# Nuralamsiddik16/Ultrafnd_git

Measured on AMD Instinct MI355X. Metric: train-step samples/sec (FakeSV batch, seq128+224^2), higher is better.
Workload: dtype bf16

## Files before the change

include/ultrafnd_hip.h:

```cpp
#ifndef ULTRAFND_HIP_H
#define ULTRAFND_HIP_H

#include <stddef.h>
#include <stdint.h>

#ifdef __cplusplus
extern "C" {
#endif

#define UFND_OK 0
#define UFND_ERR_INVALID 1
#define UFND_ERR_LAUNCH 2

#define UFND_ABI_VERSION 6

const char* ufnd_last_error(void);
int ufnd_abi_version(void);

typedef struct ufnd_step_state {
  uint64_t step;
  uint64_t seed;
  float lr;
  float weight_decay;
  float beta1, beta2, eps;
// ... 165 lines not shown
int ufnd_attention_bf16(const void* qkv, const int32_t* key_mask, void* ctx, int B, int L, int heads,
                        void* stream);

int ufnd_qkv_attention_bf16(const void* X, const void* Wqkv, const float* bqkv, const int32_t* key_mask, void* ctx, int B, int L,
                            int heads, int ldx, int ldw, const ufnd_gemm_ln* ln, void* stream);

int ufnd_text_pack(const int32_t* mask, int B, int L, int32_t* cu_seqlens, int32_t* row_src, void* stream);
int ufnd_text_pack_bins(const int32_t* mask, int B, int L, int32_t* cu_seqlens, int32_t* row_src, int32_t* bins, int32_t* nbins,
                        void* stream);
int ufnd_bert_embed_live(const int64_t* ids, const int32_t* row_src, const int* m_live, const float* word, const float* pos,
                         const float* type0, const float* gamma, const float* beta, void* x_bf16, float* x_f32, int capacity, int L,
                         int H, int vocab, float eps, void* stream);
int ufnd_gemm_bf16_live(const void* A, const void* W, const float* bias, const float* residual, void* out_bf16, float* out_f32,
                        int M, int N, int K, int lda, int ldw, int ldr, int ldo, int ldf, int act, int tile_cfg, const int* m_live,
                        void* stream);
int ufnd_gemm_bf16_ln_live(const void* A, const void* W, const float* bias, const float* residual, void* out_bf16, float* out_f32,
                           int M, int N, int K, int lda, int ldw, int ldr, int ldo, int ldf, int act, const ufnd_gemm_ln* ln,
                           const int* m_live, void* stream);
int ufnd_qkv_attention_bf16_packed(const void* X, const void* Wqkv, const float* bqkv, const int32_t* key_mask, const int32_t* cu_seqlens,
                                   void* ctx, int B, int L, int heads, int ldx, int ldw, const ufnd_gemm_ln* ln, void* stream);
int ufnd_qkv_attention_bf16_bins(const void* X, const void* Wqkv, const float* bqkv, const int32_t* key_mask, const int32_t* cu_seqlens,
                                 const int32_t* bins, const int32_t* nbins, void* ctx, int B, int L, int heads, int ldx, int ldw,
                                 const ufnd_gemm_ln* ln, void* stream);
int ufnd_attention_bf16_varlen_masked(const void* qkv, const int32_t* cu_seqlens, const int32_t* key_mask, void* ctx, int B, int max_len,
                                      int heads, void* stream);

int ufnd_qkv_attention_bf16_vit(const void* X, const void* Wqkv, const float* bqkv, void* ctx, int N, int T, int heads, int ldx, int ldw,
                                const ufnd_gemm_ln* ln, void* stream);
int ufnd_layernorm_live(const float* x, int ldx, const float* gamma, const float* beta, void* out_bf16, float* out_f32, int capacity,
                        int H, float eps, const int* m_live, void* stream);
int ufnd_masked_meanpool_l2_live(const float* hidden, const int32_t* mask, const int32_t* cu_seqlens, float* out, int B, int L, int H,
                                 void* stream);

int ufnd_bert_embed(const int64_t* ids, const float* word, const float* pos, const float* type0, const float* gamma,
                    const float* beta, void* x_bf16, float* x_f32, int B, int L, int H, int vocab, float eps,
                    void* stream);

int ufnd_masked_meanpool_l2(const float* hidden, const int32_t* mask, float* out, int B, int L, int H,
                            void* stream);

int ufnd_field_mean_l2(const float* parts, const int32_t* valid, float* out, int N, int M, int D, void* stream);

int ufnd_vit_patchify(const float* frames, void* patches_bf16, int N, int image, int patch, void* stream);

int ufnd_vit_assemble(const float* patch_emb, const float* cls, const float* pos, const float* gamma,
                      const float* beta, float* x_f32, void* x_bf16, float* stats, int N, int P, int H, float eps,
// ... 214 lines not shown
```

ultrafnd_git_amd/_lib.py:

```python
from __future__ import annotations

import ctypes as C
from pathlib import Path
from typing import Optional

import torch

_PKG = Path(__file__).resolve().parent
LIB_PATH = _PKG / "libultrafnd_hip.so"


class UltrafndHipError(RuntimeError):
    pass


class StepState(C.Structure):
    _fields_ = [("step", C.c_uint64), ("seed", C.c_uint64), ("lr", C.c_float), ("weight_decay", C.c_float),
                ("beta1", C.c_float), ("beta2", C.c_float), ("eps", C.c_float), ("max_norm", C.c_float),
                ("grad_scale", C.c_float), ("loss", C.c_float), ("grad_norm", C.c_float), ("clip_coef", C.c_float),
                ("bc1", C.c_float), ("bc2_sqrt", C.c_float), ("micro", C.c_uint32), ("reserved", C.c_float * 2)]


class Dims(C.Structure):
    _fields_ = [("hidden", C.c_int), ("text_dim", C.c_int), ("audio_dim", C.c_int), ("visual_dim", C.c_int),
# ... 127 lines not shown
                 "ufnd_softmax_ce", "ufnd_grad_norm", "ufnd_adamw_step", "ufnd_step_advance"):
        getattr(lib, name).restype = I
    _declare_encoders(lib)


def _declare_encoders(lib: C.CDLL) -> None:
    P, I, S, F = C.c_void_p, C.c_int, C.c_size_t, C.c_float
    sigs = {
        "ufnd_cast_bf16": [P, P, S, P],
        "ufnd_gemm_bf16": [P] * 6 + [I] * 9 + [P],
        "ufnd_gemm_bf16_ex": [P] * 6 + [I] * 10 + [P],
        "ufnd_layernorm": [P, I, P, P, P, P, I, I, F, P],
        "ufnd_attention_bf16": [P, P, P, I, I, I, P],
        "ufnd_qkv_attention_bf16": [P, P, P, P, P, I, I, I, I, I, C.POINTER(GemmLn), P],
        "ufnd_bert_embed": [P] * 8 + [I, I, I, I, F, P],
        "ufnd_masked_meanpool_l2": [P, P, P, I, I, I, P],
        "ufnd_text_pack": [P, I, I, P, P, P],
        "ufnd_text_pack_bins": [P, I, I, P, P, P, P, P],
        "ufnd_bert_embed_live": [P] * 10 + [I, I, I, I, F, P],
        "ufnd_gemm_bf16_live": [P] * 6 + [I] * 10 + [P, P],
        "ufnd_gemm_bf16_ln_live": [P] * 6 + [I] * 9 + [C.POINTER(GemmLn), P, P],
        "ufnd_qkv_attention_bf16_packed": [P, P, P, P, P, P, I, I, I, I, I, C.POINTER(GemmLn), P],
        "ufnd_qkv_attention_bf16_bins": [P] * 8 + [I, I, I, I, I, C.POINTER(GemmLn), P],
        "ufnd_qkv_attention_bf16_vit": [P, P, P, P, I, I, I, I, I, C.POINTER(GemmLn), P],
        "ufnd_attention_bf16_varlen_masked": [P, P, P, P, I, I, I, P],
        "ufnd_layernorm_live": [P, I, P, P, P, P, I, I, F, P, P],
        "ufnd_masked_meanpool_l2_live": [P, P, P, P, I, I, I, P],
        "ufnd_vit_patchify": [P, P, I, I, I, P],
        "ufnd_vit_assemble": [P] * 8 + [I, I, I, F, P],
        "ufnd_gemm_bf16_ln": [P] * 6 + [I] * 9 + [C.POINTER(GemmLn), P],
        "ufnd_gemm_bf16_stat_parts": [I, I, I],
        "ufnd_ln_fold_guard": [P, I, I, I, F, P, P],
        "ufnd_gemm_bf16_tile_count": [],
        "ufnd_gemm_bf16_tile_info": [I, C.POINTER(I), C.POINTER(I), C.POINTER(I)],
        "ufnd_stream_create_cu_mask": [C.POINTER(C.c_uint32), I, C.POINTER(P)],
        "ufnd_stream_destroy": [P],
        "ufnd_device_cu_count": [],
        "ufnd_l2norm_frames": [P, P, I, I, I, P],
        "ufnd_field_mean_l2": [P, P, P, I, I, I, P],
        "ufnd_temporal_align": [P] * 8 + [I] * 5 + [F, P, P],
    }
    sigs.update({
        "ufnd_gemm_bf16_dgrad": [P] * 6 + [I] * 10 + [P],
        "ufnd_gemm_bf16_wgrad": [P, P, P, I, I, I, I, I, I, P, I, P],
        "ufnd_transpose_bf16": [P, I, I, I, I, P, I, I, P, P, I, P],
        "ufnd_linear_wgrad": [P, I, P, I, I, I, I, P, P, P, P, I, P, P, C.POINTER(PartialsJob), I, P],
# ... 141 lines not shown
```

ultrafnd_git_amd/csrc/gemm_bf16.hip:

```cpp
#include "gemm_bf16_kernel.hpp"
#include "gemm_bf16_checks.hpp"

#define UFND_GEMM_TILE_PP UFND_GEMM_TILE_PERSISTENT
int ufnd_pp_pick(const void* gemm_args);
int ufnd_pp_launch(void* gemm_args, void* stream);
int ufnd_pp_stat_parts(int N);

namespace {
__global__ __launch_bounds__(256) void cast_bf16_kernel(const float* src, __bf16* dst, size_t n) {
  for (size_t i = (blockIdx.x * (size_t)256 + threadIdx.x) * 4; i < n; i += (size_t)gridDim.x * 256 * 4) {
    if (i + 4 <= n) {
      const f32x4 v = *reinterpret_cast<const f32x4*>(src + i);
      bf16x4 o = {(__bf16)v[0], (__bf16)v[1], (__bf16)v[2], (__bf16)v[3]};
      *reinterpret_cast<bf16x4*>(dst + i) = o;
    } else {
      for (size_t j = i; j < n; ++j) dst[j] = (__bf16)src[j];
    }
  }
}

}

extern "C" int ufnd_gemm_bf16_live(const void* A, const void* W, const float* bias, const float* residual, void* out_bf16,
                                   float* out_f32, int M, int N, int K, int lda, int ldw, int ldr, int ldo, int ldf, int act,
// ... 125 lines not shown
  if (ln && ln->a_stats) {
    UFND_REQUIRE(ln->colsum && ufnd_aligned(ln->colsum, 16) && ufnd_aligned(ln->a_stats, 16), "qkv_attention: colsum / a_stats alignment");
    UFND_REQUIRE(ln->a_parts >= 2 && ln->a_parts <= 24 && ln->a_parts % 2 == 0 && ln->width > 0, "qkv_attention: a_parts=%d width=%d", ln->a_parts, ln->width);
    a.a_stats = ln->a_stats; a.colsum = ln->colsum; a.a_parts = ln->a_parts; a.a_eps = ln->a_eps;
    a.inv_h = 1.0f / (float)ln->width;
    a.guard = ln->guard;
  }
  a.att_mask = key_mask;
  a.att_cu = cu_seqlens;
  a.att_bins = bins;
  a.att_nbins = nbins;
  a.m_live = cu_seqlens ? cu_seqlens + B : nullptr;
  a.att_ctx = (__bf16*)ctx;
  a.att_h = H;
  a.att_scale_log2e = 0.125f * 1.44269504088896340736f;
  a.m_tiles = B;
  a.n_tiles = heads / 2;
  a.xcd_cols = (a.n_tiles % 2 == 0 && a.m_tiles >= 4) ? 2 : 1;
  hipLaunchKernelGGL((gemm_bf16_kernel<128, 384, 2, 4, 3, 2, 16, 0, 0, 1, 1>), dim3(a.m_tiles * a.n_tiles), dim3(512), 0, (hipStream_t)stream_, a);
  UFND_CHECK_LAUNCH();
  return UFND_OK;
}

extern "C" int ufnd_qkv_attention_bf16_vit(const void* X, const void* Wqkv, const float* bqkv, void* ctx, int N, int T, int heads, int ldx,
                                           int ldw, const ufnd_gemm_ln* ln, void* stream_) {
  UFND_REQUIRE(X && Wqkv && ctx, "qkv_attention_vit: null operand");
  UFND_REQUIRE(T >= 1 && T <= 64, "qkv_attention_vit: T=%d (this kernel is built for samples of 1 to 64 rows; use ufnd_gemm_bf16[_ln] + "
               "ufnd_attention_bf16 otherwise)", T);
  UFND_REQUIRE(heads >= 1 && heads <= 64 && N >= 1 && (long long)N * T <= (1 << 24), "qkv_attention_vit: N=%d T=%d heads=%d", N, T, heads);
  const int H = heads * 64;
  UFND_REQUIRE(ldx % 8 == 0 && ldw % 8 == 0 && ldx >= H && ldw >= H && ufnd_aligned(X, 16) && ufnd_aligned(Wqkv, 16) && ufnd_aligned(ctx, 16),
               "qkv_attention_vit: strides must be multiples of 8 and pointers 16-B aligned");
  UFND_REQUIRE(!bqkv || ufnd_aligned(bqkv, 16), "qkv_attention_vit: bias alignment");
  GemmArgs a{(const __bf16*)X, (const __bf16*)Wqkv, bqkv, nullptr, nullptr, nullptr, N * T, 3 * H, H, ldx, ldw, 0, 0, 0, UFND_ACT_NONE, 0, 0, nullptr};
  if (ln && ln->a_stats) {
    UFND_REQUIRE(ln->colsum && ufnd_aligned(ln->colsum, 16) && ufnd_aligned(ln->a_stats, 16), "qkv_attention_vit: colsum / a_stats alignment");
    UFND_REQUIRE(ln->a_parts >= 2 && ln->a_parts <= 24 && ln->a_parts % 2 == 0 && ln->width > 0, "qkv_attention_vit: a_parts=%d width=%d", ln->a_parts, ln->width);
    a.a_stats = ln->a_stats; a.colsum = ln->colsum; a.a_parts = ln->a_parts; a.a_eps = ln->a_eps;
    a.inv_h = 1.0f / (float)ln->width;
    a.guard = ln->guard;
  }
  a.att_ctx = (__bf16*)ctx;
  a.att_h = H;
  a.att_t = T;
  a.att_scale_log2e = 0.125f * 1.44269504088896340736f;
  a.m_tiles = ufnd_cdiv(N, 256 / T);
// ... 23 lines not shown
```

ultrafnd_git_amd/csrc/gemm_bf16_kernel.hpp:

```cpp
#pragma once
#ifndef UFND_GEMM_OUT_NT
#define UFND_GEMM_OUT_NT 0
#endif

#include <type_traits>

#include "common.hpp"
#include "attn_softmax.hpp"

#pragma clang fp contract(off)

#ifndef UFND_GEMM_ILV
#define UFND_GEMM_ILV 1
#endif

namespace {

constexpr int BK = 64;

struct GemmArgs {
  const __bf16* A;
  const __bf16* W;
  const float* bias;
  const float* residual;
// ... 46 lines not shown

__device__ __forceinline__ bf16x8 lds_frag(const char* tile, int row, int chunk) {
  return *reinterpret_cast<const bf16x8*>(tile + row * 128 + ((chunk ^ ((row >> 1) & 7)) << 4));
}

template <int N>
__device__ __forceinline__ void wait_vmcnt() {
  static_assert(N >= 0 && N <= 63, "vmcnt range");
  asm volatile("s_waitcnt vmcnt(%0)" ::"n"(N) : "memory");
}

template <int V> struct IntC { static constexpr int value = V; };

constexpr int gemm_waves_per_simd(int BM, int BN, int WM, int WN, int STA, int STB, int MI, int LNX, int ATT) {
  const int ring = (STA * BM + STB * BN) * 128, cbytes = WM * WN * MI * (BN / WN + 4) * 4;
  const int smem = (ring > cbytes ? ring : cbytes) + (LNX ? BM * 8 + 64 : 0);
  return (!ATT && smem <= 80 * 1024 ? 2 : 1) * WM * WN / 4;
}
template <int BM, int BN, int WM, int WN, int STA, int STB, int MI, int ABL = 0, int DBG = 0, int LNX = 0, int ATT = 0, int BWD = 0>
__global__ __launch_bounds__(WM * WN * 64) __attribute__((amdgpu_waves_per_eu(gemm_waves_per_simd(BM, BN, WM, WN, STA, STB, MI, LNX, ATT))))
void gemm_bf16_kernel(const GemmArgs a) {
  static_assert(!BWD || (!LNX && !ATT && !ABL && !DBG), "backward forms are plain kernels");
  static_assert(MI == 16 || MI == 32, "MFMA shape");
  static_assert(!ATT || (((BM == 128 && BN == 384) || (BM == 256 && BN == 192)) && MI == 16 && WM * WN == 8 && LNX == 1), "fused attention tile");
  constexpr bool VIT = ATT && BM == 256;
  using acc_t = typename std::conditional<MI == 16, f32x4, f32x16>::type;
  constexpr int AR = MI * MI / 64;
  constexpr int KQ = MI == 16 ? 1 : 2;
  constexpr int NW = WM * WN;
  constexpr int TM = BM / WM, TN = BN / WN;
  constexpr int MT = TM / MI, NT = TN / MI;
  constexpr int ASLOT = BM * 128, BSLOT = BN * 128;
  constexpr int DA = STA - 1, DB = STB - 1;
  constexpr int APIECES = BM / 8, BPIECES = BN / 8;
  constexpr int PWA = APIECES / NW, PWB = (BPIECES + NW - 1) / NW;
  constexpr int WAITN = PWA * (DA - 1 > 0 ? DA - 1 : 0) + PWB * (DB - 1 > 0 ? DB - 1 : 0);
  constexpr int CP = TN + 4;
  constexpr int CBYTES = NW * MI * CP * 4;
  constexpr int RING = STA * ASLOT + STB * BSLOT;
  constexpr int ATT_OFF = (CBYTES + 1023) & ~1023;
  constexpr int ATT_IMG = BM * 128;
  constexpr int ATT_END = ATT ? ATT_OFF + (VIT ? 3 * ATT_IMG + 256 : 6 * ATT_IMG + 2048) : 0;
  constexpr int STAT_OFF0 = (RING > CBYTES) ? RING : CBYTES;
  constexpr int STAT_OFF = STAT_OFF0 > ATT_END ? STAT_OFF0 : ATT_END;
  constexpr int SMEM = STAT_OFF + (LNX ? BM * 8 + 64 : 0);
  static_assert(SMEM <= 160 * 1024, "LDS budget");
  static_assert(APIECES % NW == 0 && TM % MI == 0 && TN % MI == 0, "tile split");
  static_assert(STB >= 2 && (STA == STB || STA == STB + 1), "ring depths");
  static_assert(WAITN <= 63, "vmcnt range");
  __shared__ __attribute__((aligned(16))) char smem[SMEM];

  unsigned long long stamp[10];
  if constexpr (DBG) {
    stamp[0] = __builtin_amdgcn_s_memtime();
    stamp[1] = __builtin_amdgcn_s_memrealtime();
  }

  int mlive = a.M, m_tiles = a.m_tiles;
  if constexpr (!BWD && !ATT) {
    if (a.m_live) {
      const int v = __builtin_amdgcn_readfirstlane(*a.m_live);
      mlive = v < a.M ? (v > 0 ? v : 0) : a.M;
      m_tiles = (mlive + BM - 1) / BM;
      if ((int)blockIdx.x >= m_tiles * a.n_tiles) return;
    }
  }
  if constexpr (ATT) {
    if (a.att_bins) {
      const int v = __builtin_amdgcn_readfirstlane(*a.att_nbins);
      m_tiles = v < a.m_tiles ? (v > 0 ? v : 0) : a.m_tiles;
      if ((int)blockIdx.x >= m_tiles * a.n_tiles) return;
    }
  }
  const int nblk = m_tiles * a.n_tiles;
  int bid, kslice = 0;
  {
    const int ngrid = BWD ? nblk * (a.ksplit > 1 ? a.ksplit : 1) : nblk;
    const int q = ngrid >> 3, r = ngrid & 7, xcd = blockIdx.x & 7, idx = blockIdx.x >> 3;
    bid = (xcd < r ? xcd * (q + 1) : r * (q + 1) + (xcd - r) * q) + idx;
    if constexpr (BWD) {
      kslice = bid / nblk;
      bid -= kslice * nblk;
    }
  }
  int tm = bid / a.n_tiles, tn = bid % a.n_tiles;
  if (a.xcd_cols == 2) {
    const int nh = a.n_tiles >> 1, per_half = m_tiles * nh;
    const int half = bid / per_half, rem = bid - half * per_half;
    tm = rem / nh;
    tn = half * nh + (rem - tm * nh);
  }
  const int m0 = tm * BM, n0 = tn * BN;
  int arow0 = m0, alen = BM;
  int srow[4] = {0, 0, 0, 0}, scnt[4] = {0, 0, 0, 0}, smeta[4] = {-1, -1, -1, -1};
  const bool slots = ATT && !VIT && a.att_bins != nullptr;
  const int vit_s = VIT ? BM / a.att_t : 0, vit_st = vit_s * a.att_t;
  if constexpr (VIT) {
    arow0 = tm * vit_st;
    alen = mlive - arow0 < vit_st ? mlive - arow0 : vit_st;
  } else if constexpr (ATT) {
    if (slots) {
      const int32_t* bd = a.att_bins + (size_t)tm * 8;
#pragma unroll
      for (int j = 0; j < 4; ++j) {
        srow[j] = __builtin_amdgcn_readfirstlane(bd[2 * j]);
        smeta[j] = __builtin_amdgcn_readfirstlane(bd[2 * j + 1]);
        const int n = smeta[j] & 255, rest = n - 32 * ((smeta[j] >> 8) & 3);
        scnt[j] = smeta[j] < 0 ? 0 : (rest < 32 ? rest : 32);
      }
#pragma unroll
      for (int j = 1; j < 4; ++j) srow[j] = scnt[j] > 0 ? srow[j] : srow[0];
    } else if (a.att_cu) {
      mlive = __builtin_amdgcn_readfirstlane(*a.m_live);
      arow0 = __builtin_amdgcn_readfirstlane(a.att_cu[tm]);
      alen = __builtin_amdgcn_readfirstlane(a.att_cu[tm + 1]) - arow0;
      if (alen <= 0) return;
    }
  } else {
    alen = mlive - m0;
  }
  auto tile_row = [&](int tr) {
    if (slots) {
      const int j = tr >> 5, q = tr & 31;
      const int r0 = j == 0 ? srow[0] : j == 1 ? srow[1] : j == 2 ? srow[2] : srow[3];
      const int c = j == 0 ? scnt[0] : j == 1 ? scnt[1] : j == 2 ? scnt[2] : scnt[3];
      return r0 + (q < c ? q : (c > 0 ? c - 1 : 0));
    }
    const int gr = arow0 + tr;
    return gr < mlive ? gr : mlive - 1;
  };
  auto tile_row_live = [&](int tr) {
    if (slots) {
      const int j = tr >> 5;
      return (tr & 31) < (j == 0 ? scnt[0] : j == 1 ? scnt[1] : j == 2 ? scnt[2] : scnt[3]);
    }
    return tr < alen;
  };
  const int wave = __builtin_amdgcn_readfirstlane(threadIdx.x >> 6), lane = threadIdx.x & 63;
  const int wm = wave / WN, wn = wave % WN, fr = lane & (MI - 1), g = lane / MI;

  acc_t acc[MT][NT];
#pragma unroll
  for (int i = 0; i < MT; ++i)
#pragma unroll
    for (int j = 0; j < NT; ++j)
#pragma unroll
      for (int r = 0; r < AR; ++r) acc[i][j][r] = 0.f;

  int nk = a.K / BK, kbase = 0;
  if constexpr (BWD) {
    if (a.ksplit > 1) {
      const int per = (nk + a.ksplit - 1) / a.ksplit;
      kbase = kslice * per * BK;
      nk = nk - kslice * per < per ? nk - kslice * per : per;
    }
  }
  const int prow = lane >> 3, ppos = lane & 7;
// ... 7 lines not shown
    const int k0 = kbase + kt * BK;
#pragma unroll
    for (int ii = 0; ii < PWA; ++ii) {
      const int p = wave + NW * ii;
      const int r = 8 * p + prow;
      const int c = ppos ^ ((r >> 1) & 7);
      int gr = arow0 + r;
      gr = gr < mlive ? gr : mlive - 1;
      if constexpr (ATT) gr = arow_att[ii];
      dma16(a.A + (size_t)gr * a.lda + k0 + c * 8, buf + p * 1024);
    }
  };
  auto issueB = [&](int t, int kt) {
    char* buf = smem + STA * ASLOT + (t % STB) * BSLOT;
    const int k0 = kbase + kt * BK;
#pragma unroll
    for (int ii = 0; ii < PWB; ++ii) {
      int p = wave + NW * ii;
      if constexpr (BPIECES % NW != 0) p = p < BPIECES ? p : p - BPIECES;
      const int r = 8 * p + prow;
      const int c = ppos ^ ((r >> 1) & 7);
      int gr = n0 + r;
      gr = gr < a.N ? gr : a.N - 1;
      if constexpr (VIT) gr = (r >> 6) * a.att_h + tn * 64 + (r & 63);
      else if constexpr (ATT) gr = (r >> 7) * a.att_h + tn * 128 + (r & 127);
      dma16(a.W + (size_t)gr * a.ldw + k0 + c * 8, buf + p * 1024);
    }
  };
  constexpr int TPR = NW * 64 / BM;
  static_assert(!LNX || TPR == 2 || TPR == 4, "threads per tile row");
  constexpr int GPT = 4 / (TPR < 4 ? TPR : 4);
  f32x4 sv[GPT][3];
  f32x2* st_lds = reinterpret_cast<f32x2*>(smem + STAT_OFF);
  const float* sp = nullptr;
  if constexpr (LNX) {
    sp = a.a_stats ? a.a_stats : a.r_stats;
    if (sp) {
      const int parts = a.a_stats ? a.a_parts : a.r_parts;
      int row = arow0 + (int)threadIdx.x / TPR;
      row = row < mlive ? row : mlive - 1;
      if constexpr (ATT) row = tile_row((int)threadIdx.x / TPR);
      const f32x4* base = reinterpret_cast<const f32x4*>(sp + (size_t)row * parts * 2);
      const int nq = parts >> 1, sub = threadIdx.x % TPR;
#pragma unroll
      for (int gi = 0; gi < GPT; ++gi)
#pragma unroll
        for (int u = 0; u < 3; ++u) {
          const int q = (sub + gi * TPR) + 4 * u;
          asm volatile("global_load_dwordx4 %0, %1, off" : "=v"(sv[gi][u]) : "v"(base + (q < nq ? q : 0)) : "memory");
        }
    }
  }
  int att_mk = 1;
  if constexpr (ATT && !VIT) {
    if (slots) {
      const int j = (int)threadIdx.x >> 7, k = threadIdx.x & 127;
      const int mt = j == 0 ? smeta[0] : j == 1 ? smeta[1] : j == 2 ? smeta[2] : smeta[3];
      att_mk = mt >= 0 && k < (mt & 255);
      if (att_mk && a.att_mask) att_mk = a.att_mask[(size_t)(mt >> 10) * BM + k];
    } else if (a.att_mask && threadIdx.x < BM) {
      att_mk = a.att_mask[m0 + threadIdx.x];
    }
  }
#pragma unroll
  for (int s = 0; s < STA; ++s) {
    const int ks = s < nk ? s : nk - 1;
    if (s < STB && (LNX || s < nk)) issueB(s, ks);
    if (LNX || s < nk) issueA(s, ks);
  }

  if constexpr (LNX) {
    if (sp) {
      constexpr int NPRO = STA * PWA + STB * PWB;
      static_assert(NPRO <= 63, "vmcnt range");
      if constexpr (GPT == 1)
        asm volatile("s_waitcnt vmcnt(%3) ; STATRETIRE %0 %1 %2" : "+v"(sv[0][0]), "+v"(sv[0][1]), "+v"(sv[0][2]) : "n"(NPRO) : "memory");
      else
        asm volatile("s_waitcnt vmcnt(%6) ; STATRETIRE %0 %1 %2 %3 %4 %5" : "+v"(sv[0][0]), "+v"(sv[0][1]), "+v"(sv[0][2]), "+v"(sv[GPT - 1][0]),
                     "+v"(sv[GPT - 1][1]), "+v"(sv[GPT - 1][2]) : "n"(NPRO) : "memory");
      const int nq_ = (a.a_stats ? a.a_parts : a.r_parts) >> 1, sub_ = threadIdx.x % TPR;
      float gs[GPT], gq[GPT];
#pragma unroll
// ... 128 lines not shown
  __builtin_amdgcn_s_barrier();
  __builtin_amdgcn_sched_barrier(0);
  if constexpr (DBG) {
    stamp[2] = __builtin_amdgcn_s_memtime();
    stamp[3] = __builtin_amdgcn_s_memrealtime();
  }
  if constexpr (ABL != 1) read_half(0, IntC<0>{}, af0, bf0);
  int t = 0;
  for (; t + STA < nk; ++t) body(t, IntC<1>{}, IntC<1>{}, IntC<1>{});
  for (; t + STB < nk; ++t) body(t, IntC<0>{}, IntC<1>{}, IntC<1>{});
  for (; t + 1 < nk; ++t) body(t, IntC<0>{}, IntC<0>{}, IntC<1>{});
  body(t, IntC<0>{}, IntC<0>{}, IntC<0>{});
  __builtin_amdgcn_sched_barrier(0);
  __builtin_amdgcn_s_barrier();
  __builtin_amdgcn_sched_barrier(0);
  if constexpr (DBG) {
    stamp[4] = __builtin_amdgcn_s_memtime();
    stamp[5] = __builtin_amdgcn_s_memrealtime();
  }

  float bj[NT], csj[NT];
#pragma unroll
  for (int j = 0; j < NT; ++j) { bj[j] = 0.f; csj[j] = 0.f; }
  auto gcol = [&](int c) { return VIT ? (c >> 6) * a.att_h + tn * 64 + (c & 63) : ATT ? (c >> 7) * a.att_h + tn * 128 + (c & 127) : n0 + c; };
  if (a.bias) {
#pragma unroll
    for (int j = 0; j < NT; ++j) bj[j] = a.bias[gcol(wn * TN + j * MI + fr)];
  }
  bool fold = false, rln = false;
  if constexpr (LNX) {
    fold = a.a_stats != nullptr;
    rln = a.r_stats != nullptr;
    if (fold) {
#pragma unroll
      for (int j = 0; j < NT; ++j) csj[j] = a.colsum[gcol(wn * TN + j * MI + fr)];
    }
  }
  float* cst = reinterpret_cast<float*>(smem) + wave * MI * CP;
  float* const outf = (BWD && a.out_f32) ? a.out_f32 + (size_t)kslice * a.slab_stride : a.out_f32;
  constexpr int CPR = TN / 8;
  constexpr int CHUNKS = MI * CPR;
  constexpr int NIT = (CHUNKS + 63) / 64;
  constexpr bool FIXCOL = (64 % CPR) == 0;
  auto ld8 = [&](const float* ptr, float (&o)[8]) {
    const f32x4 x0 = *reinterpret_cast<const f32x4*>(ptr), x1 = *reinterpret_cast<const f32x4*>(ptr + 4);
#pragma unroll
    for (int q = 0; q < 4; ++q) { o[q] = x0[q]; o[4 + q] = x1[q]; }
// ... 111 lines not shown
          for (int q = 0; q < 8; ++q) v[q] = __fadd_rn(v[q], rr8[it][q]);
        }
        if constexpr (LNX && RES) {
          if (a.out_stats) {
            if constexpr (CPR % 4 == 0) {
              float sm = 0.f, sq = 0.f;
#pragma unroll
              for (int q = 0; q < 8; ++q) { sm = __fadd_rn(sm, v[q]); sq = __fmaf_rn(v[q], v[q], sq); }
              sm += quad_xor1(sm);
              sq += quad_xor1(sq);
              sm += quad_xor2(sm);
              sq += quad_xor2(sq);
              if (live && (id & 3) == 0)
                *reinterpret_cast<f32x2*>(a.out_stats + ((size_t)row * (a.N >> 5) + (col >> 5)) * 2) = f32x2{sm, sq};
            }
          }
        }
        if constexpr (ATT) {
          const int ct = wn * TN + cl;
          const int trow = wm * TM + i * MI + rr, img = ct >> 6, ch = (ct & 63) >> 3;
          bf16x8 o;
#pragma unroll
          for (int q = 0; q < 8; ++q) o[q] = (__bf16)v[q];
          const int sw = img >= (VIT ? 2 : 4) ? (ch ^ (((trow >> 1) & 3) << 1)) : (ch ^ ((trow >> 1) & 7));
          *reinterpret_cast<bf16x8*>(smem + ATT_OFF + img * ATT_IMG + trow * 128 + (sw << 4)) = o;
          continue;
        }
        if (!live) continue;
        if (a.out_f32) {
          float* op = outf + (size_t)row * a.ldf + col;
          *reinterpret_cast<f32x4*>(op) = f32x4{v[0], v[1], v[2], v[3]};
          *reinterpret_cast<f32x4*>(op + 4) = f32x4{v[4], v[5], v[6], v[7]};
        }
        if (a.out_bf16) {
          bf16x8 o;
#pragma unroll
          for (int q = 0; q < 8; ++q) o[q] = (__bf16)v[q];
          if constexpr (UFND_GEMM_OUT_NT && !BWD) __builtin_nontemporal_store(o, reinterpret_cast<bf16x8*>(a.out_bf16 + (size_t)row * a.ldo + col));
          else *reinterpret_cast<bf16x8*>(a.out_bf16 + (size_t)row * a.ldo + col) = o;
        }
      }
      asm volatile("s_waitcnt lgkmcnt(0)" ::: "memory");
    }
  };
  if constexpr (LNX) {
    if (fold) {
      if (a.act == UFND_ACT_GELU) epilogue(IntC<UFND_ACT_GELU>{}, IntC<1>{});
// ... 80 lines not shown
          uu.s2[1] = t1;
#pragma unroll
          for (int qt = 0; qt < 2; ++qt) o[dt][qt] = __builtin_amdgcn_mfma_f32_16x16x32_bf16(uu.v, pf[ksd][qt], o[dt][qt], 0, 0, 0);
        }
      }
#pragma unroll
      for (int qt = 0; qt < 2; ++qt) {
        float l = l_run[qt];
        l += __shfl_xor(l, 16, 64);
        l += __shfl_xor(l, 32, 64);
        const float inv = 1.0f / l;
        const int q = q0 + qt * 16 + f16;
        if (q >= T) continue;
        __bf16* dst = a.att_ctx + (size_t)(arow0 + r0 + q) * a.att_h + tn * 64 + 4 * g4;
#pragma unroll
        for (int dt = 0; dt < 4; ++dt) {
          bf16x4 ov = {(__bf16)(o[dt][qt][0] * inv), (__bf16)(o[dt][qt][1] * inv), (__bf16)(o[dt][qt][2] * inv), (__bf16)(o[dt][qt][3] * inv)};
          *reinterpret_cast<bf16x4*>(dst + dt * 16) = ov;
        }
      }
    }
  } else if constexpr (ATT) {
    constexpr float NEG_MASK = -3.0e38f;
    float* kbias = reinterpret_cast<float*>(smem + ATT_OFF + 6 * 16384);
    if (slots || threadIdx.x < BM) kbias[threadIdx.x] = att_mk != 0 ? 0.0f : NEG_MASK;
    __syncthreads();
    const int hh = wave >> 2, wq = wave & 3, g4 = lane >> 4, f16 = lane & 15;
    int wrow0 = arow0 + 32 * wq, wcnt = alen - 32 * wq, koff = 0;
    const float* wbias = kbias;
    if (slots) {
      const int mt = wq == 0 ? smeta[0] : wq == 1 ? smeta[1] : wq == 2 ? smeta[2] : smeta[3];
      wrow0 = wq == 0 ? srow[0] : wq == 1 ? srow[1] : wq == 2 ? srow[2] : srow[3];
      wcnt = wq == 0 ? scnt[0] : wq == 1 ? scnt[1] : wq == 2 ? scnt[2] : scnt[3];
      koff = 32 * (wq - ((mt >> 8) & 3));
      wbias = kbias + wq * BM;
    }
    const char* qimg = smem + ATT_OFF + hh * 16384;
    const char* kimg = smem + ATT_OFF + (2 + hh) * 16384;
    const char* vimg = smem + ATT_OFF + (4 + hh) * 16384;
    bf16x8 qf[2][2];
#pragma unroll
    for (int qt = 0; qt < 2; ++qt) {
      const int q = wq * 32 + qt * 16 + f16;
      qf[qt][0] = lds_frag(qimg, q, g4);
      qf[qt][1] = lds_frag(qimg, q, g4 + 4);
    }
    f32x4 o[4][2];
#pragma unroll
    for (int dt = 0; dt < 4; ++dt)
#pragma unroll
      for (int qt = 0; qt < 2; ++qt) o[dt][qt] = f32x4{0.f, 0.f, 0.f, 0.f};
    float m_run[2] = {-INFINITY, -INFINITY}, l_run[2] = {0.f, 0.f};
    constexpr int KB = 64, KT = KB / 16;
    if (wcnt > 0) {
#pragma unroll
    for (int kb0 = 0; kb0 < BM; kb0 += KB) {
      const int kr0 = koff + kb0;
      if (masked_block_is_noop(wbias + kb0, lane, m_run)) continue;
      f32x4 sc[KT][2];
#pragma unroll
      for (int kt = 0; kt < KT; ++kt)
#pragma unroll
        for (int qt = 0; qt < 2; ++qt) sc[kt][qt] = f32x4{0.f, 0.f, 0.f, 0.f};
#pragma unroll
      for (int kk = 0; kk < 2; ++kk)
#pragma unroll
        for (int kt = 0; kt < KT; ++kt) {
          const bf16x8 kf = lds_frag(kimg, (kr0 + kt * 16 + f16) & (BM - 1), g4 + 4 * kk);
#pragma unroll
          for (int qt = 0; qt < 2; ++qt) sc[kt][qt] = __builtin_amdgcn_mfma_f32_16x16x32_bf16(kf, qf[qt][kk], sc[kt][qt], 0, 0, 0);
        }
      const bool any_masked = __any(wbias[kb0 + lane] != 0.0f);
      bf16x8 pf[KT / 2][2];
#pragma unroll
      for (int qt = 0; qt < 2; ++qt) {
        const float alpha = online_softmax_block<KT>(sc, qt, wbias + kb0, any_masked, g4, a.att_scale_log2e, m_run[qt], l_run[qt], pf);
        if (!__all(alpha == 1.0f)) {
#pragma unroll
          for (int dt = 0; dt < 4; ++dt) o[dt][qt] *= alpha;
        }
      }
#pragma unroll
      for (int ksd = 0; ksd < KT / 2; ++ksd) {
#pragma unroll
        for (int dt = 0; dt < 4; ++dt) {
          const int qq = f16 >> 2, pp = f16 & 3;
          const int key0 = (kr0 + 32 * ksd + 4 * g4 + qq) & (BM - 1);
          const int ch = 2 * dt + (pp >> 1);
          const int off0 = key0 * 128 + ((ch ^ (((key0 >> 1) & 3) << 1)) << 4) + 8 * (pp & 1);
          const int key1 = key0 + 16;
          const int off1 = key1 * 128 + ((ch ^ (((key1 >> 1) & 3) << 1)) << 4) + 8 * (pp & 1);
          const s16x4 t0 = __builtin_amdgcn_ds_read_tr16_b64_v4i16((s16x4 __attribute__((address_space(3)))*)(vimg + off0));
          const s16x4 t1 = __builtin_amdgcn_ds_read_tr16_b64_v4i16((s16x4 __attribute__((address_space(3)))*)(vimg + off1));
          union { s16x4 s2[2]; bf16x8 v; } u;
          u.s2[0] = t0;
          u.s2[1] = t1;
#pragma unroll
          for (int qt = 0; qt < 2; ++qt) o[dt][qt] = __builtin_amdgcn_mfma_f32_16x16x32_bf16(u.v, pf[ksd][qt], o[dt][qt], 0, 0, 0);
        }
      }
    }
    }
#pragma unroll
    for (int qt = 0; qt < 2; ++qt) {
      float l = l_run[qt];
      l += __shfl_xor(l, 16, 64);
      l += __shfl_xor(l, 32, 64);
      const float inv = 1.0f / l;
      const int q = qt * 16 + f16;
      if (q >= wcnt) continue;
      __bf16* dst = a.att_ctx + (size_t)(wrow0 + q) * a.att_h + (tn * 2 + hh) * 64 + 4 * g4;
#pragma unroll
      for (int dt = 0; dt < 4; ++dt) {
        bf16x4 ov = {(__bf16)(o[dt][qt][0] * inv), (__bf16)(o[dt][qt][1] * inv), (__bf16)(o[dt][qt][2] * inv), (__bf16)(o[dt][qt][3] * inv)};
        *reinterpret_cast<bf16x4*>(dst + dt * 16) = ov;
      }
    }
  }
  if constexpr (LNX) {
    if (a.guard && a.a_stats && threadIdx.x == 0) {
      const float* gw = reinterpret_cast<const float*>(smem + STAT_OFF + BM * 8);
      float worst = gw[0];
#pragma unroll
      for (int w = 1; w < NW; ++w) worst = fmaxf(worst, gw[w]);
      atomicMax(reinterpret_cast<int*>(a.guard + (blockIdx.x & 1023)), __float_as_int(worst));
    }
  }
  if constexpr (DBG) {
    asm volatile("s_waitcnt vmcnt(0)" ::: "memory");
    stamp[6] = __builtin_amdgcn_s_memtime();
    stamp[7] = __builtin_amdgcn_s_memrealtime();
    if (threadIdx.x == 0) {
      constexpr int NS = ATT ? 10 : 8;
#pragma unroll
      for (int i = 0; i < NS; ++i) a.stamps[(size_t)blockIdx.x * NS + i] = stamp[i];
    }
  }
}

}

#define UFND_GEMM_TILES(X)                                                                             \
  X(0, 128, 128, 2, 2, 3, 3, 16, 0, 0)                                                              \
  X(1, 128, 64, 2, 2, 3, 3, 16, 0, 0)                                                 \
  X(2, 256, 128, 4, 2, 3, 3, 16, 1, 1)                                                              \
  X(3, 128, 128, 2, 2, 2, 2, 16, 1, 0)                                                \
  X(4, 128, 64, 2, 2, 4, 4, 16, 0, 0)                                                               \
  X(5, 256, 64, 4, 2, 3, 3, 16, 0, 0)                                                               \
  X(6, 128, 288, 2, 2, 3, 3, 16, 0, 0)                                   \
  X(7, 128, 96, 2, 2, 3, 3, 16, 0, 0)                                     \
  X(8, 256, 192, 4, 2, 2, 2, 16, 1, 1)                                  \
  X(9, 128, 384, 2, 2, 2, 2, 16, 0, 0)                                                              \
  X(10, 128, 192, 2, 2, 3, 3, 16, 0, 0)                                                             \
  X(11, 128, 96, 2, 2, 4, 4, 16, 0, 0)                                                              \
  X(12, 64, 96, 1, 2, 4, 4, 16, 0, 0)                     \
  X(13, 64, 192, 1, 2, 3, 3, 16, 0, 0)                                                              \
  X(14, 128, 256, 2, 2, 2, 2, 16, 0, 0)                                                             \
  X(15, 256, 256, 4, 2, 2, 2, 16, 1, 1)                                                             \
  X(16, 128, 128, 4, 2, 3, 3, 16, 1, 1)                                  \
  X(17, 128, 192, 4, 2, 3, 3, 16, 1, 1)                                  \
  X(18, 256, 64, 4, 2, 4, 4, 16, 0, 0)                                                              \
// ... 121 lines not shown
```

ultrafnd_git_amd/csrc/gemm_bf16_pp.hip:

```cpp
#include "gemm_bf16_pp.hpp"

__attribute__((visibility("hidden"))) int ufnd_pp_pick(const void* gemm_args) { return pp_pick(*static_cast<const GemmArgs*>(gemm_args)) ? 1 : 0; }
__attribute__((visibility("hidden"))) int ufnd_pp_stat_parts(int N) { return pp_stat_parts(N); }
__attribute__((visibility("hidden"))) int ufnd_pp_launch(void* gemm_args, void* stream) {
  GemmArgs& a = *static_cast<GemmArgs*>(gemm_args);
  if (a.out_stats && (pp_stat_parts(a.N) == 0 || !ufnd_aligned(a.out_stats, 16))) {
    ufnd_set_error("gemm_bf16 (persistent form): out_stats unsupported for this shape");
    return UFND_ERR_INVALID;
  }
  int rc = launch_pp(a, 0, (hipStream_t)stream);
  if (rc != UFND_OK) return rc;
  UFND_CHECK_LAUNCH();
  return UFND_OK;
}
```

ultrafnd_git_amd/encoders.py:

```python
from __future__ import annotations

import ctypes
import warnings
from collections import OrderedDict
from typing import Dict, NamedTuple, Optional, Tuple

import torch
import torch.nn as nn

from . import _lib as L

ACT_NONE, ACT_GELU, ACT_QUICK_GELU = 0, 1, 2


def _bf16(t: torch.Tensor) -> torch.Tensor:
    t = t.contiguous()
    out = torch.empty(t.shape, dtype=torch.bfloat16, device=t.device)
    L.check(L.lib().ufnd_cast_bf16(t.data_ptr(), out.data_ptr(), t.numel(), L.stream_ptr(t.device)), "ufnd_cast_bf16")
    return out


def dropout_prob(name: str, p) -> float:
    p = float(p)
    if not 0.0 <= p < 1.0:
# ... 163 lines not shown
        return Wp, Wp.float().sum(1).contiguous(), (b + (W * beta[None, :]).sum(1)).contiguous()

    def _ln(self, x, ldx, gamma, beta, out_bf16, out_f32, M, H, eps, m_live=None):
        if m_live is not None:
            L.check(L.lib().ufnd_layernorm_live(x.data_ptr(), ldx, gamma.data_ptr(), beta.data_ptr(), L.ptr(out_bf16),
                                                L.ptr(out_f32), M, H, eps, m_live, L.stream_ptr(x.device)), "ufnd_layernorm_live")
            return
        L.check(L.lib().ufnd_layernorm(x.data_ptr(), ldx, gamma.data_ptr(), beta.data_ptr(), L.ptr(out_bf16),
                                       L.ptr(out_f32), M, H, eps, L.stream_ptr(x.device)), "ufnd_layernorm")

    def _qkv_attn(self, A, W, bias, mask_i32, ctx, B, Lq, heads, a_stats=None, colsum=None, eps=1e-5, cu=None, bins=None, nbins=None):
        ln = None
        if a_stats is not None:
            ln = L.GemmLn()
            ln.a_stats, ln.colsum, ln.a_parts, ln.a_eps, ln.r_eps, ln.width = a_stats.data_ptr(), colsum.data_ptr(), a_stats.shape[1], eps, eps, self.hidden
            ln.guard = self._guard_buf(A.device).data_ptr()
        if Lq <= 64:
            if mask_i32 is not None or cu is not None or bins is not None:
                raise L.UltrafndHipError("_qkv_attn: the short-sample kernel (Lq <= 64) takes no key mask, cu or bins")
            L.check(L.lib().ufnd_qkv_attention_bf16_vit(A.data_ptr(), W.data_ptr(), L.ptr(bias), ctx.data_ptr(), B, Lq, heads, A.stride(0),
                                                        W.stride(0), ctypes.byref(ln) if ln is not None else None, L.stream_ptr(A.device)),
                    "ufnd_qkv_attention_bf16_vit")
            return
        L.check(L.lib().ufnd_qkv_attention_bf16_bins(A.data_ptr(), W.data_ptr(), L.ptr(bias), L.ptr(mask_i32), L.ptr(cu), L.ptr(bins),
                                                     L.ptr(nbins), ctx.data_ptr(), B, Lq, heads, A.stride(0), W.stride(0),
                                                     ctypes.byref(ln) if ln is not None else None, L.stream_ptr(A.device)),
                "ufnd_qkv_attention_bf16_bins")

    def _attn(self, qkv, mask_i32, ctx, B, Lq, heads):
        L.check(L.lib().ufnd_attention_bf16(qkv.data_ptr(), L.ptr(mask_i32), ctx.data_ptr(), B, Lq, heads,
                                            L.stream_ptr(qkv.device)), "ufnd_attention_bf16")


class _TextPass(NamedTuple):
    B: int
    Lq: int
    mask: torch.Tensor
    fuse: bool
    live: Optional[int] = None
    cu: Optional[torch.Tensor] = None
    bins: Optional[torch.Tensor] = None
    nbins: Optional[torch.Tensor] = None


class BertTextEncoder(_EncoderBase):
    def __init__(self, layers: int = 12, hidden: int = 768, heads: int = 12, intermediate: int = 3072,
                 vocab_size: int = 30522, max_position: int = 512, type_vocab: int = 2, eps: float = 1e-12,
                 fold_ln: bool = True, residual_dtype: str = "bf16", hidden_dropout_prob: float = 0.0,
# ... 345 lines not shown
```

Measured before the change: 29350.

## Fuse QKV+attention over pairs of sequence bins with one head per tile

```diff
diff --git a/include/ultrafnd_hip.h b/include/ultrafnd_hip.h
--- a/include/ultrafnd_hip.h
+++ b/include/ultrafnd_hip.h
@@ -211,6 +211,9 @@
 int ufnd_qkv_attention_bf16_bins(const void* X, const void* Wqkv, const float* bqkv, const int32_t* key_mask, const int32_t* cu_seqlens,
                                  const int32_t* bins, const int32_t* nbins, void* ctx, int B, int L, int heads, int ldx, int ldw,
                                  const ufnd_gemm_ln* ln, void* stream);
+int ufnd_qkv_attention_bf16_bin_pairs(const void* X, const void* Wqkv, const float* bqkv, const int32_t* key_mask,
+                                      const int32_t* cu_seqlens, const int32_t* bins, const int32_t* nbins, void* ctx, int B, int L,
+                                      int heads, int ldx, int ldw, const ufnd_gemm_ln* ln, void* stream);
 int ufnd_attention_bf16_varlen_masked(const void* qkv, const int32_t* cu_seqlens, const int32_t* key_mask, void* ctx, int B, int max_len,
                                       int heads, void* stream);
 
diff --git a/ultrafnd_git_amd/_lib.py b/ultrafnd_git_amd/_lib.py
--- a/ultrafnd_git_amd/_lib.py
+++ b/ultrafnd_git_amd/_lib.py
@@ -173,6 +173,7 @@
         "ufnd_gemm_bf16_ln_live": [P] * 6 + [I] * 9 + [C.POINTER(GemmLn), P, P],
         "ufnd_qkv_attention_bf16_packed": [P, P, P, P, P, P, I, I, I, I, I, C.POINTER(GemmLn), P],
         "ufnd_qkv_attention_bf16_bins": [P] * 8 + [I, I, I, I, I, C.POINTER(GemmLn), P],
+        "ufnd_qkv_attention_bf16_bin_pairs": [P] * 8 + [I, I, I, I, I, C.POINTER(GemmLn), P],
         "ufnd_qkv_attention_bf16_vit": [P, P, P, P, I, I, I, I, I, C.POINTER(GemmLn), P],
         "ufnd_attention_bf16_varlen_masked": [P, P, P, P, I, I, I, P],
         "ufnd_layernorm_live": [P, I, P, P, P, P, I, I, F, P, P],
diff --git a/ultrafnd_git_amd/csrc/gemm_bf16.hip b/ultrafnd_git_amd/csrc/gemm_bf16.hip
--- a/ultrafnd_git_amd/csrc/gemm_bf16.hip
+++ b/ultrafnd_git_amd/csrc/gemm_bf16.hip
@@ -171,6 +171,42 @@
   return UFND_OK;
 }
 
+extern "C" int ufnd_qkv_attention_bf16_bin_pairs(const void* X, const void* Wqkv, const float* bqkv, const int32_t* key_mask,
+                                                 const int32_t* cu_seqlens, const int32_t* bins, const int32_t* nbins, void* ctx, int B,
+                                                 int L, int heads, int ldx, int ldw, const ufnd_gemm_ln* ln, void* stream_) {
+  UFND_REQUIRE(X && Wqkv && ctx, "qkv_attention_bin_pairs: null operand");
+  UFND_REQUIRE(cu_seqlens && bins && nbins, "qkv_attention_bin_pairs: needs cu_seqlens, bins and nbins (ufnd_text_pack_bins)");
+  UFND_REQUIRE(L == 128 && heads >= 1 && heads <= 64 && B >= 1 && B <= 16384,
+               "qkv_attention_bin_pairs: B=%d L=%d heads=%d (this kernel is built for 128-token samples and 1 to 64 heads; "
+               "use ufnd_gemm_bf16[_ln] + ufnd_attention_bf16_varlen_masked otherwise)", B, L, heads);
+  const int H = heads * 64;
+  UFND_REQUIRE(ldx % 8 == 0 && ldw % 8 == 0 && ldx >= H && ldw >= H && ufnd_aligned(X, 16) && ufnd_aligned(Wqkv, 16) && ufnd_aligned(ctx, 16),
+               "qkv_attention_bin_pairs: strides must be multiples of 8 and pointers 16-B aligned");
+  UFND_REQUIRE(!bqkv || ufnd_aligned(bqkv, 16), "qkv_attention_bin_pairs: bias alignment");
+  GemmArgs a{(const __bf16*)X, (const __bf16*)Wqkv, bqkv, nullptr, nullptr, nullptr, B * L, 3 * H, H, ldx, ldw, 0, 0, 0, UFND_ACT_NONE, 0, 0, nullptr};
+  if (ln && ln->a_stats) {
+    UFND_REQUIRE(ln->colsum && ufnd_aligned(ln->colsum, 16) && ufnd_aligned(ln->a_stats, 16), "qkv_attention_bin_pairs: colsum / a_stats alignment");
+    UFND_REQUIRE(ln->a_parts >= 2 && ln->a_parts <= 24 && ln->a_parts % 2 == 0 && ln->width > 0, "qkv_attention_bin_pairs: a_parts=%d width=%d", ln->a_parts, ln->width);
+    a.a_stats = ln->a_stats; a.colsum = ln->colsum; a.a_parts = ln->a_parts; a.a_eps = ln->a_eps;
+    a.inv_h = 1.0f / (float)ln->width;
+    a.guard = ln->guard;
+  }
+  a.att_mask = key_mask;
+  a.att_cu = cu_seqlens;
+  a.att_bins = bins;
+  a.att_nbins = nbins;
+  a.m_live = cu_seqlens + B;
+  a.att_ctx = (__bf16*)ctx;
+  a.att_h = H;
+  a.att_scale_log2e = 0.125f * 1.44269504088896340736f;
+  a.m_tiles = ufnd_cdiv(B, 2);
+  a.n_tiles = heads;
+  a.xcd_cols = (a.n_tiles % 2 == 0 && a.m_tiles >= 4) ? 2 : 1;
+  hipLaunchKernelGGL((gemm_bf16_kernel<256, 192, 4, 2, 3, 2, 16, 0, 0, 1, 2>), dim3(a.m_tiles * a.n_tiles), dim3(512), 0, (hipStream_t)stream_, a);
+  UFND_CHECK_LAUNCH();
+  return UFND_OK;
+}
+
 extern "C" int ufnd_qkv_attention_bf16_vit(const void* X, const void* Wqkv, const float* bqkv, void* ctx, int N, int T, int heads, int ldx,
                                            int ldw, const ufnd_gemm_ln* ln, void* stream_) {
   UFND_REQUIRE(X && Wqkv && ctx, "qkv_attention_vit: null operand");
diff --git a/ultrafnd_git_amd/csrc/gemm_bf16_kernel.hpp b/ultrafnd_git_amd/csrc/gemm_bf16_kernel.hpp
--- a/ultrafnd_git_amd/csrc/gemm_bf16_kernel.hpp
+++ b/ultrafnd_git_amd/csrc/gemm_bf16_kernel.hpp
@@ -92,8 +92,12 @@
 void gemm_bf16_kernel(const GemmArgs a) {
   static_assert(!BWD || (!LNX && !ATT && !ABL && !DBG), "backward forms are plain kernels");
   static_assert(MI == 16 || MI == 32, "MFMA shape");
-  static_assert(!ATT || (((BM == 128 && BN == 384) || (BM == 256 && BN == 192)) && MI == 16 && WM * WN == 8 && LNX == 1), "fused attention tile");
-  constexpr bool VIT = ATT && BM == 256;
+  static_assert(!ATT || (((ATT == 1 && BM == 128 && BN == 384) || (BM == 256 && BN == 192)) && MI == 16 && WM * WN == 8 && LNX == 1), "fused attention tile");
+  static_assert(ATT >= 0 && ATT <= 2, "fused attention geometry");
+  constexpr bool VIT = ATT == 1 && BM == 256;
+  constexpr bool PAIR = ATT == 2;
+  constexpr bool HEAD1 = VIT || PAIR;
+  constexpr int NSL = PAIR ? 8 : 4;
   using acc_t = typename std::conditional<MI == 16, f32x4, f32x16>::type;
   constexpr int AR = MI * MI / 64;
   constexpr int KQ = MI == 16 ? 1 : 2;
@@ -110,7 +114,7 @@
   constexpr int RING = STA * ASLOT + STB * BSLOT;
   constexpr int ATT_OFF = (CBYTES + 1023) & ~1023;
   constexpr int ATT_IMG = BM * 128;
-  constexpr int ATT_END = ATT ? ATT_OFF + (VIT ? 3 * ATT_IMG + 256 : 6 * ATT_IMG + 2048) : 0;
+  constexpr int ATT_END = ATT ? ATT_OFF + (VIT ? 3 * ATT_IMG + 256 : PAIR ? 3 * ATT_IMG + 4096 : 6 * ATT_IMG + 2048) : 0;
   constexpr int STAT_OFF0 = (RING > CBYTES) ? RING : CBYTES;
   constexpr int STAT_OFF = STAT_OFF0 > ATT_END ? STAT_OFF0 : ATT_END;
   constexpr int SMEM = STAT_OFF + (LNX ? BM * 8 + 64 : 0);
@@ -126,7 +130,7 @@
     stamp[1] = __builtin_amdgcn_s_memrealtime();
   }
 
-  int mlive = a.M, m_tiles = a.m_tiles;
+  int mlive = a.M, m_tiles = a.m_tiles, nbins = 0;
   if constexpr (!BWD && !ATT) {
     if (a.m_live) {
       const int v = __builtin_amdgcn_readfirstlane(*a.m_live);
@@ -138,7 +142,12 @@
   if constexpr (ATT) {
     if (a.att_bins) {
       const int v = __builtin_amdgcn_readfirstlane(*a.att_nbins);
-      m_tiles = v < a.m_tiles ? (v > 0 ? v : 0) : a.m_tiles;
+      if constexpr (PAIR) {
+        nbins = v < (a.M >> 7) ? (v > 0 ? v : 0) : (a.M >> 7);
+        m_tiles = (nbins + 1) >> 1;
+      } else {
+        m_tiles = v < a.m_tiles ? (v > 0 ? v : 0) : a.m_tiles;
+      }
       if ((int)blockIdx.x >= m_tiles * a.n_tiles) return;
     }
   }
@@ -162,24 +171,33 @@
   }
   const int m0 = tm * BM, n0 = tn * BN;
   int arow0 = m0, alen = BM;
-  int srow[4] = {0, 0, 0, 0}, scnt[4] = {0, 0, 0, 0}, smeta[4] = {-1, -1, -1, -1};
-  const bool slots = ATT && !VIT && a.att_bins != nullptr;
+  int srow[NSL], scnt[NSL], smeta[NSL];
+#pragma unroll
+  for (int j = 0; j < NSL; ++j) { srow[j] = 0; scnt[j] = 0; smeta[j] = -1; }
+#define UFND_SLOT_OF(v, j)                                                                                                        \
+  (NSL == 8 ? ((j) == 0 ? v[0] : (j) == 1 ? v[1] : (j) == 2 ? v[2] : (j) == 3 ? v[3] : (j) == 4 ? v[NSL - 4] : (j) == 5 ? v[NSL - 3] \
+                                                                                                : (j) == 6   ? v[NSL - 2]         \
+                                                                                                             : v[NSL - 1])        \
+            : ((j) == 0 ? v[0] : (j) == 1 ? v[1] : (j) == 2 ? v[2] : v[3]))
+  const bool slots = PAIR || (ATT && !VIT && a.att_bins != nullptr);
   const int vit_s = VIT ? BM / a.att_t : 0, vit_st = vit_s * a.att_t;
   if constexpr (VIT) {
     arow0 = tm * vit_st;
     alen = mlive - arow0 < vit_st ? mlive - arow0 : vit_st;
   } else if constexpr (ATT) {
     if (slots) {
-      const int32_t* bd = a.att_bins + (size_t)tm * 8;
-#pragma unroll
-      for (int j = 0; j < 4; ++j) {
-        srow[j] = __builtin_amdgcn_readfirstlane(bd[2 * j]);
-        smeta[j] = __builtin_amdgcn_readfirstlane(bd[2 * j + 1]);
+#pragma unroll
+      for (int j = 0; j < NSL; ++j) {
+        const int bin = PAIR ? 2 * tm + (j >> 2) : tm;
+        const bool have = !PAIR || bin < nbins;
+        const int32_t* bd = a.att_bins + (size_t)(have ? bin : 2 * tm) * 8;
+        srow[j] = __builtin_amdgcn_readfirstlane(bd[2 * (j & 3)]);
+        smeta[j] = have ? __builtin_amdgcn_readfirstlane(bd[2 * (j & 3) + 1]) : -1;
         const int n = smeta[j] & 255, rest = n - 32 * ((smeta[j] >> 8) & 3);
         scnt[j] = smeta[j] < 0 ? 0 : (rest < 32 ? rest : 32);
       }
 #pragma unroll
-      for (int j = 1; j < 4; ++j) srow[j] = scnt[j] > 0 ? srow[j] : srow[0];
+      for (int j = 1; j < NSL; ++j) srow[j] = scnt[j] > 0 ? srow[j] : srow[0];
     } else if (a.att_cu) {
       mlive = __builtin_amdgcn_readfirstlane(*a.m_live);
       arow0 = __builtin_amdgcn_readfirstlane(a.att_cu[tm]);
@@ -192,8 +210,7 @@
   auto tile_row = [&](int tr) {
     if (slots) {
       const int j = tr >> 5, q = tr & 31;
-      const int r0 = j == 0 ? srow[0] : j == 1 ? srow[1] : j == 2 ? srow[2] : srow[3];
-      const int c = j == 0 ? scnt[0] : j == 1 ? scnt[1] : j == 2 ? scnt[2] : scnt[3];
+      const int r0 = UFND_SLOT_OF(srow, j), c = UFND_SLOT_OF(scnt, j);
       return r0 + (q < c ? q : (c > 0 ? c - 1 : 0));
     }
     const int gr = arow0 + tr;
@@ -201,8 +218,7 @@
   };
   auto tile_row_live = [&](int tr) {
     if (slots) {
-      const int j = tr >> 5;
-      return (tr & 31) < (j == 0 ? scnt[0] : j == 1 ? scnt[1] : j == 2 ? scnt[2] : scnt[3]);
+      return (tr & 31) < UFND_SLOT_OF(scnt, tr >> 5);
     }
     return tr < alen;
   };
@@ -256,7 +272,7 @@
       const int c = ppos ^ ((r >> 1) & 7);
       int gr = n0 + r;
       gr = gr < a.N ? gr : a.N - 1;
-      if constexpr (VIT) gr = (r >> 6) * a.att_h + tn * 64 + (r & 63);
+      if constexpr (HEAD1) gr = (r >> 6) * a.att_h + tn * 64 + (r & 63);
       else if constexpr (ATT) gr = (r >> 7) * a.att_h + tn * 128 + (r & 127);
       dma16(a.W + (size_t)gr * a.ldw + k0 + c * 8, buf + p * 1024);
     }
@@ -285,13 +301,18 @@
         }
     }
   }
-  int att_mk = 1;
+  int att_mk = 1, att_mk2 = 1;
   if constexpr (ATT && !VIT) {
     if (slots) {
       const int j = (int)threadIdx.x >> 7, k = threadIdx.x & 127;
-      const int mt = j == 0 ? smeta[0] : j == 1 ? smeta[1] : j == 2 ? smeta[2] : smeta[3];
+      const int mt = UFND_SLOT_OF(smeta, j);
       att_mk = mt >= 0 && k < (mt & 255);
-      if (att_mk && a.att_mask) att_mk = a.att_mask[(size_t)(mt >> 10) * BM + k];
+      if (att_mk && a.att_mask) att_mk = a.att_mask[(size_t)(mt >> 10) * 128 + k];
+      if constexpr (PAIR) {
+        const int mt2 = UFND_SLOT_OF(smeta, 4 + j);
+        att_mk2 = mt2 >= 0 && k < (mt2 & 255);
+        if (att_mk2 && a.att_mask) att_mk2 = a.att_mask[(size_t)(mt2 >> 10) * 128 + k];
+      }
     } else if (a.att_mask && threadIdx.x < BM) {
       att_mk = a.att_mask[m0 + threadIdx.x];
     }
@@ -466,7 +487,7 @@
   float bj[NT], csj[NT];
 #pragma unroll
   for (int j = 0; j < NT; ++j) { bj[j] = 0.f; csj[j] = 0.f; }
-  auto gcol = [&](int c) { return VIT ? (c >> 6) * a.att_h + tn * 64 + (c & 63) : ATT ? (c >> 7) * a.att_h + tn * 128 + (c & 127) : n0 + c; };
+  auto gcol = [&](int c) { return HEAD1 ? (c >> 6) * a.att_h + tn * 64 + (c & 63) : ATT ? (c >> 7) * a.att_h + tn * 128 + (c & 127) : n0 + c; };
   if (a.bias) {
 #pragma unroll
     for (int j = 0; j < NT; ++j) bj[j] = a.bias[gcol(wn * TN + j * MI + fr)];
@@ -624,7 +645,7 @@
           bf16x8 o;
 #pragma unroll
           for (int q = 0; q < 8; ++q) o[q] = (__bf16)v[q];
-          const int sw = img >= (VIT ? 2 : 4) ? (ch ^ (((trow >> 1) & 3) << 1)) : (ch ^ ((trow >> 1) & 7));
+          const int sw = img >= (HEAD1 ? 2 : 4) ? (ch ^ (((trow >> 1) & 3) << 1)) : (ch ^ ((trow >> 1) & 7));
           *reinterpret_cast<bf16x8*>(smem + ATT_OFF + img * ATT_IMG + trow * 128 + (sw << 4)) = o;
           continue;
         }
@@ -751,22 +772,25 @@
     }
   } else if constexpr (ATT) {
     constexpr float NEG_MASK = -3.0e38f;
+    constexpr int LK = 128;
     float* kbias = reinterpret_cast<float*>(smem + ATT_OFF + 6 * 16384);
-    if (slots || threadIdx.x < BM) kbias[threadIdx.x] = att_mk != 0 ? 0.0f : NEG_MASK;
+    if (slots || threadIdx.x < LK) kbias[threadIdx.x] = att_mk != 0 ? 0.0f : NEG_MASK;
+    if constexpr (PAIR) kbias[NW * 64 + threadIdx.x] = att_mk2 != 0 ? 0.0f : NEG_MASK;
     __syncthreads();
     const int hh = wave >> 2, wq = wave & 3, g4 = lane >> 4, f16 = lane & 15;
     int wrow0 = arow0 + 32 * wq, wcnt = alen - 32 * wq, koff = 0;
     const float* wbias = kbias;
     if (slots) {
-      const int mt = wq == 0 ? smeta[0] : wq == 1 ? smeta[1] : wq == 2 ? smeta[2] : smeta[3];
-      wrow0 = wq == 0 ? srow[0] : wq == 1 ? srow[1] : wq == 2 ? srow[2] : srow[3];
-      wcnt = wq == 0 ? scnt[0] : wq == 1 ? scnt[1] : wq == 2 ? scnt[2] : scnt[3];
+      const int ws = PAIR ? wave : wq;
+      const int mt = UFND_SLOT_OF(smeta, ws);
+      wrow0 = UFND_SLOT_OF(srow, ws);
+      wcnt = UFND_SLOT_OF(scnt, ws);
       koff = 32 * (wq - ((mt >> 8) & 3));
-      wbias = kbias + wq * BM;
+      wbias = kbias + ws * LK;
     }
     const char* qimg = smem + ATT_OFF + hh * 16384;
-    const char* kimg = smem + ATT_OFF + (2 + hh) * 16384;
-    const char* vimg = smem + ATT_OFF + (4 + hh) * 16384;
+    const char* kimg = smem + ATT_OFF + (PAIR ? 1 * ATT_IMG : 2 * 16384) + hh * 16384;
+    const char* vimg = smem + ATT_OFF + (PAIR ? 2 * ATT_IMG : 4 * 16384) + hh * 16384;
     bf16x8 qf[2][2];
 #pragma unroll
     for (int qt = 0; qt < 2; ++qt) {
@@ -783,7 +807,7 @@
     constexpr int KB = 64, KT = KB / 16;
     if (wcnt > 0) {
 #pragma unroll
-    for (int kb0 = 0; kb0 < BM; kb0 += KB) {
+    for (int kb0 = 0; kb0 < LK; kb0 += KB) {
       const int kr0 = koff + kb0;
       if (masked_block_is_noop(wbias + kb0, lane, m_run)) continue;
       f32x4 sc[KT][2];
@@ -795,7 +819,7 @@
       for (int kk = 0; kk < 2; ++kk)
 #pragma unroll
         for (int kt = 0; kt < KT; ++kt) {
-          const bf16x8 kf = lds_frag(kimg, (kr0 + kt * 16 + f16) & (BM - 1), g4 + 4 * kk);
+          const bf16x8 kf = lds_frag(kimg, (kr0 + kt * 16 + f16) & (LK - 1), g4 + 4 * kk);
 #pragma unroll
           for (int qt = 0; qt < 2; ++qt) sc[kt][qt] = __builtin_amdgcn_mfma_f32_16x16x32_bf16(kf, qf[qt][kk], sc[kt][qt], 0, 0, 0);
         }
@@ -814,7 +838,7 @@
 #pragma unroll
         for (int dt = 0; dt < 4; ++dt) {
           const int qq = f16 >> 2, pp = f16 & 3;
-          const int key0 = (kr0 + 32 * ksd + 4 * g4 + qq) & (BM - 1);
+          const int key0 = (kr0 + 32 * ksd + 4 * g4 + qq) & (LK - 1);
           const int ch = 2 * dt + (pp >> 1);
           const int off0 = key0 * 128 + ((ch ^ (((key0 >> 1) & 3) << 1)) << 4) + 8 * (pp & 1);
           const int key1 = key0 + 16;
@@ -838,7 +862,7 @@
       const float inv = 1.0f / l;
       const int q = qt * 16 + f16;
       if (q >= wcnt) continue;
-      __bf16* dst = a.att_ctx + (size_t)(wrow0 + q) * a.att_h + (tn * 2 + hh) * 64 + 4 * g4;
+      __bf16* dst = a.att_ctx + (size_t)(wrow0 + q) * a.att_h + (PAIR ? tn : tn * 2 + hh) * 64 + 4 * g4;
 #pragma unroll
       for (int dt = 0; dt < 4; ++dt) {
         bf16x4 ov = {(__bf16)(o[dt][qt][0] * inv), (__bf16)(o[dt][qt][1] * inv), (__bf16)(o[dt][qt][2] * inv), (__bf16)(o[dt][qt][3] * inv)};
@@ -866,6 +890,8 @@
     }
   }
 }
+
+#undef UFND_SLOT_OF
 
 }
 
diff --git a/ultrafnd_git_amd/csrc/gemm_bf16_pp.hip b/ultrafnd_git_amd/csrc/gemm_bf16_pp.hip
--- a/ultrafnd_git_amd/csrc/gemm_bf16_pp.hip
+++ b/ultrafnd_git_amd/csrc/gemm_bf16_pp.hip
@@ -1,4 +1,5 @@
 #include "gemm_bf16_pp.hpp"
+#include "gemm_bf16_checks.hpp"
 
 __attribute__((visibility("hidden"))) int ufnd_pp_pick(const void* gemm_args) { return pp_pick(*static_cast<const GemmArgs*>(gemm_args)) ? 1 : 0; }
 __attribute__((visibility("hidden"))) int ufnd_pp_stat_parts(int N) { return pp_stat_parts(N); }
@@ -8,6 +9,13 @@
     ufnd_set_error("gemm_bf16 (persistent form): out_stats unsupported for this shape");
     return UFND_ERR_INVALID;
   }
+  if (a.out_stats) {
+    const int one_tile = stat_parts_for(auto_cfg(a.M, a.N, a.K), a.N);
+    if (one_tile != 0 && one_tile != pp_stat_parts(a.N)) {
+      ufnd_set_error("gemm_bf16 (persistent form): %d statistics partials per row, the one-tile form of this shape writes %d", pp_stat_parts(a.N), one_tile);
+      return UFND_ERR_INVALID;
+    }
+  }
   int rc = launch_pp(a, 0, (hipStream_t)stream);
   if (rc != UFND_OK) return rc;
   UFND_CHECK_LAUNCH();
diff --git a/ultrafnd_git_amd/encoders.py b/ultrafnd_git_amd/encoders.py
--- a/ultrafnd_git_amd/encoders.py
+++ b/ultrafnd_git_amd/encoders.py
@@ -209,8 +209,14 @@
                                                         W.stride(0), ctypes.byref(ln) if ln is not None else None, L.stream_ptr(A.device)),
                     "ufnd_qkv_attention_bf16_vit")
             return
-        L.check(L.lib().ufnd_qkv_attention_bf16_bins(A.data_ptr(), W.data_ptr(), L.ptr(bias), L.ptr(mask_i32), L.ptr(cu), L.ptr(bins),
-                                                     L.ptr(nbins), ctx.data_ptr(), B, Lq, heads, A.stride(0), W.stride(0),
+        if bins is not None:
+            L.check(L.lib().ufnd_qkv_attention_bf16_bin_pairs(A.data_ptr(), W.data_ptr(), L.ptr(bias), L.ptr(mask_i32), L.ptr(cu), L.ptr(bins),
+                                                              L.ptr(nbins), ctx.data_ptr(), B, Lq, heads, A.stride(0), W.stride(0),
+                                                              ctypes.byref(ln) if ln is not None else None, L.stream_ptr(A.device)),
+                    "ufnd_qkv_attention_bf16_bin_pairs")
+            return
+        L.check(L.lib().ufnd_qkv_attention_bf16_bins(A.data_ptr(), W.data_ptr(), L.ptr(bias), L.ptr(mask_i32), L.ptr(cu), None,
+                                                     None, ctx.data_ptr(), B, Lq, heads, A.stride(0), W.stride(0),
                                                      ctypes.byref(ln) if ln is not None else None, L.stream_ptr(A.device)),
                 "ufnd_qkv_attention_bf16_bins")
 
```

Result: no change. 29590, median of 6 (+0.8%).
